# tuanggolt/hyperdrive

Measured on AMD Instinct MI355X. Metric: verified consensus msgs/sec (secp256k1) at 1/2/4/8 MI355X; % INT32 VALU peak, higher is better.
Workload: dtype u32 (256-bit modular integer arithmetic)

## Files before the change

### hyperdrive_amd/_lib.py

```python
from __future__ import annotations

import atexit
import ctypes
import os
import weakref

HERE = os.path.dirname(os.path.abspath(__file__))
LIB_PATH = os.environ.get("HD_LIB", os.path.join(HERE, "_lib", "libhdverify.so"))

HD_OK = 0
HD_EINVAL = -1
HD_ENOMEM = -2
HD_EDEVICE = -3
HD_ECAP = -4
HD_EAGAIN = -5

c_u8p = ctypes.POINTER(ctypes.c_uint8)
c_i8p = ctypes.POINTER(ctypes.c_int8)
c_i64p = ctypes.POINTER(ctypes.c_int64)
c_u32p = ctypes.POINTER(ctypes.c_uint32)
c_i32p = ctypes.POINTER(ctypes.c_int32)


class HdBatch(ctypes.Structure):
# ... 144 lines not shown
class HdMqTaken(ctypes.Structure):
    _fields_ = [("n", ctypes.c_uint32), ("removed", ctypes.c_uint32), ("batch", HdBatch),
                ("d_sender", ctypes.c_void_p), ("d_valid_bitmap", ctypes.c_void_p), ("d_value_ok", ctypes.c_void_p),
                ("n_proposes", ctypes.c_uint32), ("proposes", ctypes.c_void_p)]


class HdTallyTicket(ctypes.Structure):
    _fields_ = [("stage", ctypes.c_void_p), ("stage_cap", ctypes.c_size_t), ("dup", ctypes.c_int),
                ("n", ctypes.c_uint32), ("H", ctypes.c_uint32), ("Cg", ctypes.c_uint32), ("need", ctypes.c_size_t),
                ("done", ctypes.c_void_p)]


SIGNATURES = {
    "hd_ctx_create": (ctypes.c_int, [ctypes.c_int, ctypes.POINTER(ctypes.c_void_p)]),
    "hd_ctx_destroy": (ctypes.c_int, [ctypes.c_void_p]),
    "hd_ctx_set_pubkey_format": (ctypes.c_int, [ctypes.c_void_p, ctypes.c_int]),
    "hd_set_signatories": (ctypes.c_int, [ctypes.c_void_p, ctypes.c_void_p, ctypes.c_uint32]),
    "hd_import_keys": (ctypes.c_int, [ctypes.c_void_p, ctypes.c_void_p, ctypes.c_uint32, ctypes.c_void_p,
                                      ctypes.c_void_p]),
    "hd_export_keys": (ctypes.c_int, [ctypes.c_void_p, ctypes.c_void_p, ctypes.c_void_p, ctypes.c_uint32,
                                      ctypes.POINTER(ctypes.c_uint32)]),
    "hd_ctx_set_change_info": (ctypes.c_int, [ctypes.c_void_p, ctypes.POINTER(HdSetChangeInfo)]),
    "hd_ctx_set_fastpath": (ctypes.c_int, [ctypes.c_void_p, ctypes.c_int]),
    "hd_ctx_fastpath_stats": (ctypes.c_int, [ctypes.c_void_p, ctypes.POINTER(ctypes.c_uint32),
                                             ctypes.POINTER(ctypes.c_uint32)]),
    "hd_ctx_foreign_stats": (ctypes.c_int, [ctypes.c_void_p, ctypes.POINTER(ctypes.c_uint32),
                                            ctypes.POINTER(ctypes.c_uint32), ctypes.POINTER(ctypes.c_uint32)]),
    "hd_ctx_dedup_stats": (ctypes.c_int, [ctypes.c_void_p, ctypes.POINTER(ctypes.c_uint64),
                                          ctypes.POINTER(ctypes.c_uint64)]),
    "hd_ctx_preimage_stats": (ctypes.c_int, [ctypes.c_void_p, ctypes.POINTER(ctypes.c_uint64),
                                             ctypes.POINTER(ctypes.c_uint64)]),
    "hd_ctx_overlap_stats": (ctypes.c_int, [ctypes.c_void_p, ctypes.POINTER(ctypes.c_uint32),
                                            ctypes.POINTER(ctypes.c_uint32), ctypes.POINTER(ctypes.c_uint32)]),
    "hd_ctx_fastpath_geometry": (ctypes.c_int, [ctypes.c_void_p, ctypes.POINTER(ctypes.c_int),
                                                ctypes.POINTER(ctypes.c_int), ctypes.POINTER(ctypes.c_int)]),
    "hd_ctx_profile": (ctypes.c_int, [ctypes.c_void_p, ctypes.c_int]),
    "hd_ctx_set_variant": (ctypes.c_int, [ctypes.c_void_p, ctypes.c_int, ctypes.c_int]),
    "hd_ctx_get_variant": (ctypes.c_int, [ctypes.c_void_p, ctypes.c_int, ctypes.POINTER(ctypes.c_int)]),
    "hd_ctx_profile_read": (ctypes.c_int, [ctypes.c_void_p, ctypes.POINTER(ctypes.c_uint32),
                                           ctypes.POINTER(ctypes.c_double), ctypes.POINTER(ctypes.c_uint32),
                                           ctypes.POINTER(ctypes.c_double)]),
    "hd_verify_batch": (ctypes.c_int, [ctypes.c_void_p, ctypes.POINTER(HdBatch), ctypes.c_void_p,
                                       ctypes.c_void_p, ctypes.c_void_p]),
    "hd_verify_batch_device": (ctypes.c_int, [ctypes.c_void_p, ctypes.POINTER(HdBatch), ctypes.c_void_p,
                                              ctypes.c_void_p, ctypes.c_void_p, ctypes.c_void_p, ctypes.c_void_p]),
    "hd_authenticate_batch_device": (ctypes.c_int, [ctypes.c_void_p, ctypes.POINTER(HdBatch), ctypes.c_void_p,
                                                    ctypes.c_void_p]),
    "hd_verify_submit": (ctypes.c_int, [ctypes.c_void_p, ctypes.POINTER(HdBatch), ctypes.c_void_p, ctypes.c_void_p,
                                        ctypes.c_void_p, ctypes.POINTER(ctypes.c_uint64)]),
    "hd_verify_submit_compact": (ctypes.c_int, [ctypes.c_void_p, ctypes.POINTER(HdBatchCompact), ctypes.c_void_p,
                                                ctypes.c_void_p, ctypes.c_void_p, ctypes.POINTER(ctypes.c_uint64)]),
    "hd_verify_wait": (ctypes.c_int, [ctypes.c_void_p, ctypes.c_uint64]),
    "hd_host_alloc": (ctypes.c_int, [ctypes.c_size_t, ctypes.POINTER(ctypes.c_void_p)]),
    "hd_host_free": (ctypes.c_int, [ctypes.c_void_p]),
    "hd_stream_create_dedicated": (ctypes.c_int, [ctypes.c_void_p, ctypes.POINTER(ctypes.c_void_p)]),
    "hd_stream_destroy": (ctypes.c_int, [ctypes.c_void_p, ctypes.c_void_p]),
    "hd_tally": (ctypes.c_int, [ctypes.c_void_p, ctypes.POINTER(HdBatch), ctypes.c_void_p,
                                ctypes.POINTER(HdTallyOut)]),
    "hd_tally_device": (ctypes.c_int, [ctypes.c_void_p, ctypes.POINTER(HdBatch), ctypes.c_void_p,
                                       ctypes.POINTER(HdTallyOut), ctypes.c_void_p]),
    "hd_tally_device_bitmap_part": (ctypes.c_int, [ctypes.c_void_p, ctypes.POINTER(HdBatch), ctypes.c_void_p,
                                                   ctypes.c_uint32, ctypes.c_uint32, ctypes.POINTER(HdTallyOut),
                                                   ctypes.c_void_p]),
    "hd_tally_partition_of": (ctypes.c_uint32, [ctypes.c_int64, ctypes.c_int64, ctypes.c_uint32]),
    "hd_tally_device_bitmap": (ctypes.c_int, [ctypes.c_void_p, ctypes.POINTER(HdBatch), ctypes.c_void_p,
                                              ctypes.POINTER(HdTallyOut), ctypes.c_void_p]),
# ... 209 lines not shown
```

### hyperdrive_amd/csrc/hd_fastverify.hip

```cpp
#include <hip/hip_runtime.h>

#include <algorithm>
#include <cstdio>
#include <cstdlib>
#include <cstring>
#include <string>
#include <map>
#include <mutex>
#include <unordered_map>
#include <vector>

#include "../../include/hd_verify.h"
#include "../../include/hd_mathcheck.h"
#include "hd_fixedbase.h"
#include "hd_dedup.h"
#include "hd_scmont.h"
#include "hd_internal.h"
#include "hd_keycarry.h"
#include "hd_verify_msg.h"

using namespace hd;

struct FbWork {
    const gp* gtab = nullptr;
    uint32_t nslots = 0;
    uint32_t max_slots = 0;
    gp** tabs = nullptr;
    std::vector<gp*> chunks;
    ge* base = nullptr;
    ge* pub = nullptr;
    uint32_t* state = nullptr;
    int32_t* adm_slot = nullptr;
    bool map_ok = true;
    size_t cap_adm_slot = 0;
    uint32_t* list = nullptr;
    uint32_t* counts = nullptr;
    uint32_t* zr = nullptr;
    struct Scratch {
        uint32_t* rows = nullptr;
        size_t cap_rows = 0;
        uint32_t* dtab = nullptr;
        size_t cap_dtab = 0;
        uint8_t* pre = nullptr;
        size_t cap_pre = 0;
        uint32_t* slow = nullptr;
        size_t cap_slow = 0;
        uint32_t* count = nullptr;
        uint32_t* slow2 = nullptr;
        size_t cap_slow2 = 0;
        hipEvent_t done = nullptr;
        hipStream_t stream = nullptr;
        bool used = false;
    };
    static constexpr int NSCRATCH = 3;
    Scratch sc[NSCRATCH];
    int next = 0;
    int last_set = -1;
    uint32_t* nr_host = nullptr;
    uint32_t* nr_dev = nullptr;
    uint32_t* est_host = nullptr;
    uint32_t* est_dev = nullptr;
    unsigned long long* dstats = nullptr;
    unsigned long long* pstats = nullptr;
    hipEvent_t done = nullptr;
    hipStream_t last = nullptr;
    bool any = false;
    bool steady = false;
    struct SumsChain {
        hipEvent_t done = nullptr;
        hipStream_t last = nullptr;
        bool prev = false, now = false;
        void begin_call() { prev = now; now = false; }
        bool wait(hipStream_t s) {
            if (!done && hipEventCreateWithFlags(&done, hipEventDisableTiming) != hipSuccess) done = nullptr;
            return done && prev && last != s && hipStreamWaitEvent(s, done, 0) == hipSuccess;
        }
        void record(hipStream_t s) {
            now = done && hipEventRecord(done, s) == hipSuccess;
            if (now) last = s;
        }
    } sums;
    uint32_t n_capped = 0, n_lean = 0, n_chained = 0;
    bool prof = false;
    std::vector<hipEvent_t> ev_call, ev_sums;
    size_t n_call = 0, n_sums = 0;
    std::unordered_map<std::string, uint32_t> slot_of;
    std::vector<uint32_t> free_slots;
    hd_set_change_info change{0, 0, 0, 0, 0};
    uint32_t used = 1;
    int wp = HD_FB_W;
    int last_k = 8;
    double budget = 0;
    size_t bytes = 0;
    uint32_t* fdict = nullptr;
    uint32_t* fnext = nullptr;
    uint32_t fbase = 0, fcap = 0, fres = 0;
    uint32_t* fpend_host = nullptr;
    uint32_t* fpend_dev = nullptr;
    uint32_t fseen = 0;
    uint32_t* fhit = nullptr;
    ge* fkey = nullptr;
    uint32_t fwait = 1, fcalls = 0;
    bool fforce = false;
    uint32_t evictions = 0;
    uint32_t evict_checks = 0;
    uint32_t evict_aborts = 0;
};

namespace {

#define FBCHK(expr, what)                                \
    do {                                                 \
        hipError_t e_ = (expr);                          \
        if (e_ != hipSuccess) return hd_ctx_fail(ctx, e_, what); \
    } while (0)

struct FastSrc {
    const DevBatch& b;
    uint32_t i;
    const uint8_t* dg;
    __device__ __forceinline__ uint32_t type() const { return b.type[i]; }
    __device__ __forceinline__ uint32_t value(int w) const { return load_be32(b.value32 + 32 * (size_t)i + 4 * w); }
    __device__ __forceinline__ uint32_t from(int w) const { return load_be32(b.from32 + 32 * (size_t)i + 4 * w); }
    __device__ __forceinline__ uint32_t sig_r(int w) const { return load_be32(b.sig65 + 65 * (size_t)i + 4 * w); }
    __device__ __forceinline__ uint32_t sig_s(int w) const { return load_be32(b.sig65 + 65 * (size_t)i + 32 + 4 * w); }
    __device__ __forceinline__ uint32_t sig_v() const { return b.sig65[65 * (size_t)i + 64]; }
    __device__ __forceinline__ void sig(uint32_t r_be[8], uint32_t s_be[8], uint32_t& v) const {
        load_sig65(r_be, s_be, v, b.sig65, i, b.n);
    }
    __device__ __forceinline__ void from_words(uint32_t w[8]) const { load_row32_be(w, b.from32, i); }
    __device__ __forceinline__ void value_words(uint32_t w[8]) const { load_row32_be(w, b.value32, i); }
};

#define HD_FAST_LIVE 0xFDu

template <int NW>
HD void soa_load(uint32_t (&w)[NW], const uint32_t* __restrict__ p, uint32_t n, uint32_t i) {
    HD_UNROLL for (int k = 0; k < NW; k++) w[k] = p[(size_t)k * n + i];
}
template <int NW>
HD void soa_store(uint32_t* __restrict__ p, uint32_t n, uint32_t i, const uint32_t (&w)[NW]) {
    HD_UNROLL for (int k = 0; k < NW; k++) p[(size_t)k * n + i] = w[k];
}

struct SplitRows {
    uint32_t* aux;
    int32_t* idx;
    uint32_t* ref;
    uint32_t* u1;
    uint32_t* u2;
    uint32_t* s;
    uint32_t* pre;
    uint32_t* xyz;
    uint32_t* cnt;
    int prio;
};

HD uint32_t dd_resolve(const SplitRows& rows, uint32_t i, uint32_t& c, bool& has_slot) {
    uint32_t rf = rows.ref[i];
    has_slot = (rf >> 30) != 3u;
    c = 0;
    if (!has_slot) return rf & 0xFFu;
    if (rf & HD_DD_REPEAT) rf = rows.ref[rf & HD_DD_INDEX];
    c = rf;
    return rows.aux[c] & 0xFFu;
}

HD void wave_prio(int p) {
    if (p == 1) __builtin_amdgcn_s_setprio(1);
    else if (p == 2) __builtin_amdgcn_s_setprio(2);
    else if (p >= 3) __builtin_amdgcn_s_setprio(3);
}

#define HD_REF_NEG 0x80000000u
#define HD_REF_ZERO 0x40000000u
#define HD_REF_IDX 0x3FFFFFFFu
// ... 198 lines not shown
            }
        }
    }
    const bool live = code == HD_FAST_LIVE;
    const bool distinct = live && rep == HD_DD_EMPTY;
    __shared__ uint32_t s_cnt[4], s_base;
    const uint32_t lane = threadIdx.x & 63u, wv = threadIdx.x >> 6;
    const unsigned long long bd = __ballot(distinct), br = __ballot(live && !distinct);
    if (lane == 0) s_cnt[wv] = (uint32_t)__popcll(bd) | (uint32_t)__popcll(br) << 16;
    __syncthreads();
    if (threadIdx.x == 0) {
        const uint32_t t = s_cnt[0] + s_cnt[1] + s_cnt[2] + s_cnt[3];
        s_base = 0;
        if (t)
            s_base = (uint32_t)atomicAdd((unsigned long long*)(rows.cnt + 2),
                                         (unsigned long long)(t & 0xFFFFu) | (unsigned long long)(t >> 16) << 32);
    }
    __syncthreads();
    if (!present) return;
    if (distinct) {
        uint32_t c = s_base + (uint32_t)__popcll(bd & ((1ull << lane) - 1ull));
        for (uint32_t w = 0; w < wv; w++) c += s_cnt[w] & 0xFFFFu;
        rows.aux[c] = slot << 8 | HD_FAST_LIVE;
        soa_store(rows.u1, n, c, m.v);
        soa_store(rows.u2, n, c, r.v);
        soa_store(rows.s, n, c, s.v);
        rows.ref[i] = c;
    } else {
        rows.ref[i] = live ? (HD_DD_REPEAT | rep) : (HD_DD_FINAL | code);
    }
    rows.idx[i] = idx;
}

template <int K>
HD uint32_t split_lanes(uint32_t nc) {
    return ((nc + (uint32_t)K - 1) / (uint32_t)K + 63u) & ~63u;
}

template <int K>
__global__ __launch_bounds__(256) void k_fast_sinv(uint32_t n, SplitRows rows, uint32_t* __restrict__ est,
                                                   unsigned long long* __restrict__ stats) {
    wave_prio(rows.prio);
    const uint32_t t = blockIdx.x * blockDim.x + threadIdx.x;
    const uint32_t nc = rows.cnt[2], T = split_lanes<K>(nc);
    if (t == 0) {
        const uint32_t reps = rows.cnt[3];
        if (est) {
            est[1] = n;
            est[0] = nc;
        }
        if (nc + reps) atomicAdd(&stats[0], (unsigned long long)nc + reps);
        if (reps) atomicAdd(&stats[1], (unsigned long long)reps);
    }
    if (t >= T) return;
    sc sv[K];
    uint32_t live = 0;
    static_for<K>([&](auto jc) {
        constexpr int j = decltype(jc)::value;
        const uint32_t i = (uint32_t)j * T + t;
        const uint32_t ic = i < nc ? i : nc - 1;
        const uint32_t a = rows.aux[ic];
        soa_load(sv[j].v, rows.s, n, ic);
        live |= (i < nc && (a & 0xFFu) == HD_FAST_LIVE) ? 1u << j : 0u;
    });
    if (!live) return;
    sm pre[K], acc;
    HD_UNROLL for (int k = 0; k < 9; k++) acc.n[k] = 0;
    static_for<K>([&](auto jc) {
        constexpr int j = decltype(jc)::value;
        if ((live >> j) & 1u) {
// ... 260 lines not shown
    const uint32_t* zrow = rows.xyz + 18 * (size_t)n;
    uint32_t live = 0;
    fe acc;
    HD_UNROLL for (int k = 0; k < 9; k++) acc.n[k] = 0;
    HD_NOUNROLL for (int j = 0; j < K; j++) {
        const uint32_t i = (uint32_t)j * T + t;
        if (!lean_live(rows, nc, i)) continue;
        fe z;
        soa_load(z.n, zrow, n, i);
        if (live) fe_mul(acc, acc, z);
        else acc = z;
        live |= 1u << j;
        soa_store(rows.pre, n, i, acc.n);
    }
    if (!live) return;
    fe inv;
    fe_inv_divsteps(inv, acc);
    HD_NOUNROLL for (int j = K - 1; j >= 0; j--) {
        if (!((live >> j) & 1u)) continue;
        const uint32_t i = (uint32_t)j * T + t;
        const uint32_t below = live & ((1u << j) - 1u);
        if (below) {
            const uint32_t ip = (uint32_t)(31 - __clz((int)below)) * T + t;
            fe pp, zi, z;
            soa_load(pp.n, rows.pre, n, ip);
            soa_load(z.n, zrow, n, i);
            fe_mul(zi, inv, pp);
            fe_mul(inv, inv, z);
            soa_store(rows.pre, n, i, zi.n);
        } else {
            soa_store(rows.pre, n, i, inv.n);
        }
    }
}

HD void fast_rx(fe& x, const sc& r, uint32_t v) {
    uint32_t xw[8];
    HD_UNROLL for (int k = 0; k < 8; k++) xw[k] = r.v[k];
    if (v & 2) {
        const uint32_t N[8] = {HD_N0, HD_N1, HD_N2, HD_N3, HD_N4, 0xFFFFFFFFu, 0xFFFFFFFFu, 0xFFFFFFFFu};
        uint64_t c = 0;
        HD_UNROLL for (int k = 0; k < 8; k++) { c += (uint64_t)xw[k] + N[k]; xw[k] = (uint32_t)c; c >>= 32; }
    }
    fe_from_le(x, xw);
}

__device__ __forceinline__ void cmp_one(const DevBatch& b, const SplitRows& rows, const int32_t* __restrict__ adm_perm,
                       uint8_t* __restrict__ verdict, uint8_t* __restrict__ rec32, int32_t* __restrict__ signer,
                       uint32_t* __restrict__ slow, uint32_t* __restrict__ n_slow, uint32_t* __restrict__ bitmap,
                       bool auth, uint32_t i, bool present, const fe* zi) {
    const uint32_t n = b.n;
    uint8_t v = HD_NEEDS_SLOW;
    if (present) {
        uint32_t c;
        bool has_slot;
        v = (uint8_t)dd_resolve(rows, i, c, has_slot);
        if (v == HD_FAST_LIVE) {
            fe xn, yn, w, x;
            soa_load(xn.n, rows.xyz, n, c);
            soa_load(yn.n, rows.xyz + 9 * (size_t)n, n, c);
            if (zi) w = *zi;
            else soa_load(w.n, rows.pre, n, c);
            sc r;
            soa_load(r.v, rows.u2, n, c);
            const uint32_t sv = b.sig65[65 * (size_t)i + 64];
            fast_rx(x, r, sv);
// ... 483 lines not shown
    gp** tp = nullptr;
    ge *base = nullptr, *pub = nullptr;
    uint32_t* cl = nullptr;
    FBCHK(hipMalloc(&tab, sizeof(gp) * (size_t)FbL<HD_FB_WG>::TAB), "G table");
    FBCHK(hipMalloc(&tp, sizeof(gp*)), "G table pointer");
    FBCHK(hipMalloc(&base, sizeof(ge) * FbL<HD_FB_WG>::NWIN), "G bases");
    FBCHK(hipMalloc(&pub, sizeof(ge)), "G point");
    FBCHK(hipMalloc(&cl, 8), "G list");
    const uint32_t hl[2] = {0u, 1u};
    hipStream_t s = ctx->stream;
    FBCHK(hipMemcpyAsync(pub, &g, sizeof(ge), hipMemcpyHostToDevice, s), "G point");
    FBCHK(hipMemcpyAsync(cl, hl, 8, hipMemcpyHostToDevice, s), "G list");
    FBCHK(hipMemcpyAsync(tp, &tab, sizeof(gp*), hipMemcpyHostToDevice, s), "G table pointer");
    k_fb_bases<HD_FB_WG><<<1, 64, 0, s>>>(cl, cl + 1, pub, base);
    k_fb_runs<HD_FB_WG><<<fb_run_blocks(ctx), 256, 0, s>>>(cl, cl + 1, base, tp, ctx->fb->zr);
    FBCHK(hipGetLastError(), "G table kernels");
    FBCHK(hipStreamSynchronize(s), "G table build");
    (void)hipFree(base);
    (void)hipFree(pub);
    (void)hipFree(cl);
    (void)hipFree(tp);
    g_fb_g_tables[ctx->device] = tab;
    *out = tab;
    return HD_OK;
}

int hd_fb_init(hd_ctx* ctx) {
    if (ctx->fb) return HD_OK;
    ctx->fb = new (std::nothrow) FbWork();
    if (!ctx->fb) return HD_ENOMEM;
    FbWork* f = ctx->fb;
    f->budget = 64.0 * (1ull << 30);
    if (const char* m = getenv("HD_FB_MAX_BYTES")) f->budget = atof(m);
    f->max_slots = (uint32_t)std::max(1.0, std::min(1e6, f->budget / fb_slot_bytes(f->wp)));
    FBCHK(hipMalloc(&f->counts, 8), "fb counts");
    FBCHK(hipMalloc(&f->zr, fb_run_scratch_bytes(ctx)), "fb builder scratch");
    FBCHK(hipHostMalloc((void**)&f->nr_host, 4, hipHostMallocMapped | hipHostMallocCoherent), "fb ready count");
    *f->nr_host = 0xFFFFFFFFu;
    FBCHK(hipHostGetDevicePointer((void**)&f->nr_dev, f->nr_host, 0), "fb ready count map");
    FBCHK(hipHostMalloc((void**)&f->est_host, 16, hipHostMallocMapped | hipHostMallocCoherent), "fb list estimate");
    f->est_host[0] = f->est_host[1] = f->est_host[2] = f->est_host[3] = 0xFFFFFFFFu;
    FBCHK(hipHostGetDevicePointer((void**)&f->est_dev, f->est_host, 0), "fb list estimate map");
    FBCHK(hipHostMalloc((void**)&f->fpend_host, 8, hipHostMallocMapped | hipHostMallocCoherent), "fb foreign claims");
    f->fpend_host[0] = f->fpend_host[1] = 0;
    FBCHK(hipHostGetDevicePointer((void**)&f->fpend_dev, f->fpend_host, 0), "fb foreign claims map");
    FBCHK(hipMalloc(&f->dstats, 16), "fb repeat counters");
    FBCHK(hipMemset(f->dstats, 0, 16), "fb repeat counters clear");
    FBCHK(hipMalloc(&f->pstats, 16), "fb preimage counters");
    FBCHK(hipMemset(f->pstats, 0, 16), "fb preimage counters clear");
    int rc = fb_alloc_slots(ctx);
    if (rc) return rc;
    return fb_g_table(ctx, &f->gtab);
}

const gp* hd_fb_gtab(const hd_ctx* ctx) { return ctx && ctx->fb ? ctx->fb->gtab : nullptr; }

void hd_fb_release(hd_ctx* ctx) {
    if (!ctx || !ctx->fb) return;
    FbWork* f = ctx->fb;
    fb_free_tables(ctx);
    if (f->done) (void)hipEventDestroy(f->done);
    if (f->sums.done) (void)hipEventDestroy(f->sums.done);
    for (hipEvent_t e : f->ev_call) (void)hipEventDestroy(e);
    for (hipEvent_t e : f->ev_sums) (void)hipEventDestroy(e);
    for (auto& sc : f->sc) {
        if (sc.done) (void)hipEventDestroy(sc.done);
        void* sp[] = {sc.rows, sc.slow, sc.count, sc.slow2, sc.dtab, sc.pre};
        for (void* p : sp)
            if (p) (void)hipFree(p);
    }
    void* ptrs[] = {f->counts, f->adm_slot, f->zr, f->fdict, f->fnext, f->fhit, f->fkey, f->dstats, f->pstats};
    for (void* p : ptrs)
        if (p) (void)hipFree(p);
    if (f->nr_host) (void)hipHostFree(f->nr_host);
    if (f->est_host) (void)hipHostFree(f->est_host);
    if (f->fpend_host) (void)hipHostFree(f->fpend_host);
    delete f;
    ctx->fb = nullptr;
}

static double fb_free_cap(hd_ctx* ctx) {
    size_t fr = 0, tot = 0;
    (void)hipSetDevice(ctx->device);
    if (hipMemGetInfo(&fr, &tot) != hipSuccess) return 1e300;
    return 0.9 * (double)fr + (double)ctx->fb->bytes;
}

static int fb_pick_width(hd_ctx* ctx, uint32_t m, int cap) {
    if (ctx->var[HD_VAR_KEY_WIDTH]) return ctx->var[HD_VAR_KEY_WIDTH];
    FbWork* f = ctx->fb;
    const double others = (double)(fb_device_bytes(ctx->device) - std::min(fb_device_bytes(ctx->device), f->bytes));
    const double free_cap = fb_free_cap(ctx);
    const double shared = std::min(f->budget - others, free_cap);
    const double slots = (double)m + 1 + (ctx->var[HD_VAR_FOREIGN_KEYS] > 0 ? ctx->var[HD_VAR_FOREIGN_KEYS] : 0);
    const auto allowed = [cap](int w) { return cap == 0 || w <= cap; };
    if (allowed(HD_FB_WX) && fb_slot_bytes(HD_FB_WX) * slots <= shared) return HD_FB_WX;
    if (allowed(HD_FB_WW) && fb_slot_bytes(HD_FB_WW) * ((double)m + 1) <= shared) return HD_FB_WW;
    if (allowed(HD_FB_W) && fb_slot_bytes(HD_FB_W) * slots <= std::min(f->budget, free_cap)) return HD_FB_W;
    return HD_FB_WN;
}
// ... 261 lines not shown
static void launch_sums(const FbCallPlan& p, uint32_t blocks, hipStream_t s, uint32_t n, const gp* gtab,
                        const gp* const* tab, const SplitRows& rows) {
    const size_t cap = p.capped ? sums_cap_lds<WP>() : 0;
    if (p.sums_pf == 2) {
        if (p.sums_waves == 2) k_fast_sums<2, WP, 2><<<blocks, 256, 0, s>>>(n, gtab, tab, rows);
        else k_fast_sums<3, WP, 2><<<blocks, 256, cap, s>>>(n, gtab, tab, rows);
    } else {
        if (p.sums_waves == 2) k_fast_sums<2, WP, 1><<<blocks, 256, 0, s>>>(n, gtab, tab, rows);
        else if (p.sums_waves == 4) k_fast_sums<4, WP, 0><<<blocks, 256, 0, s>>>(n, gtab, tab, rows);
        else k_fast_sums<3, WP, 1><<<blocks, 256, cap, s>>>(n, gtab, tab, rows);
    }
}

template <int K, int WP>
static void launch_split(hd_ctx* ctx, const DevBatch& b, const uint8_t* d_digest, uint8_t* d_verdict,
                         uint8_t* d_rec32, int32_t* d_signer, uint32_t* d_bitmap, const SplitRows& rows,
                         const FbWork::Scratch& sc, hipStream_t s, bool auth, const FbCallPlan& p) {
    FbWork* f = ctx->fb;
    const uint32_t n = b.n;
    const uint32_t tb = (split_lanes<K>(n) + 255) / 256, nb = (n + 255) / 256;
    const uint32_t tw = dd_table_words(n);
    uint32_t* dtab = p.dedup ? sc.dtab : nullptr;
    const uint32_t* fdict = f->fcap ? f->fdict : nullptr;
    if (p.share) {
        const PreRows pre{sc.pre, (uint32_t*)(sc.pre + 32 * (size_t)n), (uint32_t*)(sc.pre + 36 * (size_t)n), sc.count};
        k_pre_claim<<<(n + HD_PRE_BLOCK - 1) / HD_PRE_BLOCK, HD_PRE_BLOCK, 0, s>>>(b, pre, sc.dtab + tw, tw - 1u, rows.prio);
        k_pre_hash<<<nb, 256, 0, s>>>(b, pre, f->pstats, rows.prio);
        k_fast_prep<true><<<nb, 256, 0, s>>>(b, nullptr, f->state, f->adm_slot, hd_adm_index(ctx), ctx->n_adm, rows,
                                             fdict, f->fhit, f->fbase, dtab, tw - 1u, pre);
    } else {
        k_fast_prep<false><<<nb, 256, 0, s>>>(b, d_digest, f->state, f->adm_slot, hd_adm_index(ctx), ctx->n_adm, rows,
                                              fdict, f->fhit, f->fbase, dtab, tw - 1u, PreRows{});
    }
    if (p.lean) k_fast_sinv_lean<K><<<tb, 256, 0, s>>>(n, rows, f->est_dev + 2, f->dstats);
    else k_fast_sinv<K><<<tb, 256, 0, s>>>(n, rows, f->est_dev + 2, f->dstats);
    if (p.chain && f->sums.wait(s)) f->n_chained++;
    hipEvent_t* pe = fb_prof_pair(f->ev_sums, f->n_sums, f->prof);
    if (pe) (void)hipEventRecord(pe[0], s);
    launch_sums<WP>(p, nb, s, n, f->gtab, f->tabs, rows);
    if (pe) (void)hipEventRecord(pe[1], s);
    if (p.chain) f->sums.record(s);
    if (p.lean) k_fast_zinv_lean<K><<<tb, 256, 0, s>>>(n, rows);
    else k_fast_zinv<K><<<tb, 256, 0, s>>>(n, rows);
    k_fast_cmp<<<nb, 256, 0, s>>>(b, rows, ctx->d_adm_perm, d_verdict, d_rec32, d_signer, sc.slow, sc.count,
                                  d_bitmap, auth);
}

static int fb_verify_impl(hd_ctx* ctx, const DevBatch& b, const uint8_t* d_digest, uint8_t* d_verdict,
                          uint8_t* d_rec32, int32_t* d_signer, uint32_t* d_bitmap, FbWork::Scratch& sc,
                          hipStream_t s, bool auth);

int hd_fb_verify(hd_ctx* ctx, const DevBatch& b, const uint8_t* d_digest, uint8_t* d_verdict, uint8_t* d_rec32,
                 int32_t* d_signer, uint32_t* d_bitmap, hipStream_t s, bool auth) {
    FbWork* f = ctx->fb;
    f->sums.begin_call();
    if (!f->done) FBCHK(hipEventCreateWithFlags(&f->done, hipEventDisableTiming), "fb event");
    const int j = f->next;
    f->next = (j + 1) % FbWork::NSCRATCH;
    FbWork::Scratch& sc = f->sc[j];
    if (!sc.done) FBCHK(hipEventCreateWithFlags(&sc.done, hipEventDisableTiming), "fb scratch event");
    if (!sc.count) FBCHK(hipMalloc(&sc.count, 32), "fb scratch count");
    bool evicted = false;
    int re = fb_evict(ctx, &evicted);
    if (re) return re;
    const bool steady = !evicted && f->nr_host && *(volatile uint32_t*)f->nr_host == 0 && !fb_foreign_pending(f);
    if (sc.used && sc.stream != s) FBCHK(hipStreamWaitEvent(s, sc.done, 0), "fb scratch order");
    if (f->any && f->last != s && !(steady && f->steady)) FBCHK(hipStreamWaitEvent(s, f->done, 0), "fb stream order");
    hipEvent_t* pe = fb_prof_pair(f->ev_call, f->n_call, f->prof);
    if (pe) (void)hipEventRecord(pe[0], s);
    const int rc = fb_verify_impl(ctx, b, d_digest, d_verdict, d_rec32, d_signer, d_bitmap, sc, s, auth);
    if (pe) (void)hipEventRecord(pe[1], s);
    FBCHK(hipEventRecord(sc.done, s), "fb scratch record");
    FBCHK(hipEventRecord(f->done, s), "fb event record");
    sc.used = true;
    sc.stream = s;
    f->last_set = j;
// ... 15 lines not shown
static int fb_verify_impl(hd_ctx* ctx, const DevBatch& b, const uint8_t* d_digest, uint8_t* d_verdict,
                          uint8_t* d_rec32, int32_t* d_signer, uint32_t* d_bitmap, FbWork::Scratch& sc,
                          hipStream_t s, bool auth) {
    FbWork* f = ctx->fb;
    int rc = hd_dev_grow(ctx, (void**)&sc.slow, &sc.cap_slow, 4 * (size_t)b.n);
    if (rc) return rc;
    const uint32_t blocks = (b.n + 255) / 256;
    rc = hd_dev_grow(ctx, (void**)&sc.slow2, &sc.cap_slow2, 4 * (size_t)b.n);
    if (rc) return rc;
    FBCHK(hipMemsetAsync(sc.count, 0, 32, s), "fb count reset");
    if (ctx->n_adm > 0 && f->adm_slot && f->map_ok) {
        if (b.n > HD_DD_MAX_N) {
            ctx->last_error = "known-key check: more than 2^30 messages in one call";
            return HD_EINVAL;
        }
        const size_t row_words = 63;
        rc = hd_dev_grow(ctx, (void**)&sc.rows, &sc.cap_rows, 4 * row_words * (size_t)b.n);
        if (rc) return rc;
        const uint32_t n = b.n;
        const volatile uint32_t* est = f->est_host;
        const FbCallPlan p = fb_plan_call(FbPlanIn{ctx->var, ctx->n_cu, n, auth, d_digest != nullptr,
                                                   {est[0], est[1], est[2], est[3]}});
        if (p.dedup || p.share) {
            const size_t tab_bytes = 4 * (size_t)dd_table_words(n);
            rc = hd_dev_grow(ctx, (void**)&sc.dtab, &sc.cap_dtab, 2 * tab_bytes);
            if (rc) return rc;
            const size_t first = p.dedup ? 0 : tab_bytes, last = p.share ? 2 * tab_bytes : tab_bytes;
            FBCHK(hipMemsetAsync((uint8_t*)sc.dtab + first, 0xFF, last - first, s), "fb table clear");
        }
        if (p.share) {
            rc = hd_dev_grow(ctx, (void**)&sc.pre, &sc.cap_pre, 40 * (size_t)n);
            if (rc) return rc;
        }
        SplitRows rows;
        rows.aux = sc.rows;
        rows.idx = (int32_t*)(sc.rows + (size_t)n);
        rows.u1 = sc.rows + 2 * (size_t)n;
        rows.u2 = sc.rows + 10 * (size_t)n;
        rows.s = sc.rows + 18 * (size_t)n;
        rows.pre = sc.rows + 26 * (size_t)n;
        rows.xyz = sc.rows + 35 * (size_t)n;
        rows.ref = sc.rows + 62 * (size_t)n;
        rows.cnt = sc.count;
        rows.prio = ctx->var[HD_VAR_WAVE_PRIO];
        with_width(f->wp, [&](auto wp) {
            with_k(p.k, [&](auto k) {
                launch_split<decltype(k)::value, decltype(wp)::value>(ctx, b, d_digest, d_verdict, d_rec32, d_signer,
                                                                      d_bitmap, rows, sc, s, auth, p);
            });
        });
        f->last_k = p.k;
        f->n_capped += p.capped;
        f->n_lean += p.lean;
        FBCHK(hipGetLastError(), "split check launch");
        if (p.lift) {
            k_slow_lift<<<p.lift_blocks, 256, 0, s>>>(b, sc.slow, sc.count, d_verdict, d_rec32, d_signer, sc.slow2,
                                                      sc.count + 1, rows.prio, f->est_dev, rows, f->gtab);
            FBCHK(hipGetLastError(), "k_slow_lift");
        }
        const SlowCtl ctl{p.lift ? sc.slow2 : sc.slow, p.lift ? sc.count + 1 : sc.count, f->adm_slot, f->state, f->pub,
                          d_bitmap, p.lift ? f->est_dev + 1 : f->est_dev, rows.prio,
                          f->fcap ? f->fdict : nullptr, f->fnext, f->fbase, f->fcap, f->fpend_dev,
                          f->fcap ? f->fhit + 64 : nullptr, f->fkey, f->fpend_dev + 1};
        rc = hd_launch_slow(ctx, b, d_digest, d_verdict, d_rec32, d_signer, nullptr, ctl, p.slow_blocks, s);
        if (rc) return rc;
        return fb_learn(ctx, s);
// ... 112 lines not shown
int hd_ctx_set_change_info(hd_ctx* ctx, hd_set_change_info* out) {
    if (!ctx || !out) return HD_EINVAL;
    *out = ctx->fb && ctx->fastpath ? ctx->fb->change : hd_set_change_info{0, 0, 0, 0, 0};
    return HD_OK;
}

int hd_ctx_dedup_stats(hd_ctx* ctx, uint64_t* checked, uint64_t* repeats) {
    if (!ctx) return HD_EINVAL;
    if (checked) *checked = 0;
    if (repeats) *repeats = 0;
    if (!ctx->fb || !ctx->fb->dstats) return HD_OK;
    (void)hipSetDevice(ctx->device);
    int rq = hd_ctx_quiesce(ctx);
    if (rq) return rq;
    unsigned long long st[2] = {0, 0};
    FBCHK(hipMemcpy(st, ctx->fb->dstats, 16, hipMemcpyDeviceToHost), "repeat counters read");
    if (checked) *checked = st[0];
    if (repeats) *repeats = st[1];
    return HD_OK;
}

int hd_ctx_preimage_stats(hd_ctx* ctx, uint64_t* typed, uint64_t* distinct) {
    if (!ctx) return HD_EINVAL;
    if (typed) *typed = 0;
    if (distinct) *distinct = 0;
    if (!ctx->fb || !ctx->fb->pstats) return HD_OK;
    (void)hipSetDevice(ctx->device);
    int rq = hd_ctx_quiesce(ctx);
    if (rq) return rq;
    unsigned long long st[2] = {0, 0};
    FBCHK(hipMemcpy(st, ctx->fb->pstats, 16, hipMemcpyDeviceToHost), "preimage counters read");
    if (typed) *typed = st[0];
    if (distinct) *distinct = st[1];
    return HD_OK;
}

int hd_ctx_overlap_stats(hd_ctx* ctx, uint32_t* capped, uint32_t* lean, uint32_t* chained) {
    if (!ctx) return HD_EINVAL;
    const FbWork* f = ctx->fb;
    if (capped) *capped = f ? f->n_capped : 0;
    if (lean) *lean = f ? f->n_lean : 0;
    if (chained) *chained = f ? f->n_chained : 0;
    return HD_OK;
}

int hd_fb_table_read(hd_ctx* ctx, int32_t which, uint64_t first, uint32_t count, uint8_t* out64, int* width,
                     uint32_t* state, uint8_t* key64) {
    if (!ctx || !ctx->fb || which < -1 || (count && !out64)) return HD_EINVAL;
    (void)hipSetDevice(ctx->device);
    FbWork* f = ctx->fb;
    int rq = hd_fb_quiesce(ctx);
    if (rq) return rq;
    FBCHK(hipStreamSynchronize(ctx->stream), "table read sync");
    const gp* tab = nullptr;
    uint64_t entries = 0;
    uint32_t st = HD_FB_READY;
    int w = HD_FB_WG;
    gp key;
    if (which < 0) {
        ge g;
        const uint32_t GX[8] = {0x79BE667Eu, 0xF9DCBBACu, 0x55A06295u, 0xCE870B07u,
                                0x029BFCDBu, 0x2DCE28D9u, 0x59F2815Bu, 0x16F81798u};
        const uint32_t GY[8] = {0x483ADA77u, 0x26A3C465u, 0x5DA4FBFCu, 0x0E1108A8u,
                                0xFD17B448u, 0xA6855419u, 0x9C47D08Fu, 0xFB10D4B8u};
        fe_from_be(g.x, GX);
        fe_from_be(g.y, GY);
// ... 37 lines not shown
```

### hyperdrive_amd/verify.py

```python
from __future__ import annotations

import ctypes
from dataclasses import dataclass
from typing import Dict, List, Optional, Sequence, Tuple

import numpy as np

from . import _lib
from ._lib import HDError, HdBatch, HdTallyOut

VALID = 0
BAD_RECID = 1
BAD_RS = 2
NO_POINT = 3
INFINITY = 4
SIGNATORY_MISMATCH = 5
NOT_ADMITTED = 6
BAD_TYPE = 7
NOT_AUTHENTIC = 8
VERDICT_NAMES = ["VALID", "BAD_RECID", "BAD_RS", "NO_POINT", "INFINITY", "SIGNATORY_MISMATCH",
                 "NOT_ADMITTED", "BAD_TYPE", "NOT_AUTHENTIC"]

PROPOSE, PREVOTE, PRECOMMIT = 1, 2, 3

# ... 726 lines not shown
        self._check(self._lib.hd_ctx_profile_read(self._ctx, ctypes.byref(c), ctypes.byref(vm), ctypes.byref(s),
                                                  ctypes.byref(sm)), "hd_ctx_profile_read")
        return c.value, vm.value, s.value, sm.value

    def fastpath_stats(self) -> Tuple[int, int]:
        k, f = ctypes.c_uint32(), ctypes.c_uint32()
        self._check(self._lib.hd_ctx_fastpath_stats(self._ctx, ctypes.byref(k), ctypes.byref(f)),
                    "hd_ctx_fastpath_stats")
        return int(k.value), int(f.value)

    def foreign_stats(self, checks: bool = False):
        r, e, c = ctypes.c_uint32(), ctypes.c_uint32(), ctypes.c_uint32()
        self._check(self._lib.hd_ctx_foreign_stats(self._ctx, ctypes.byref(r), ctypes.byref(e), ctypes.byref(c)),
                    "hd_ctx_foreign_stats")
        return (int(r.value), int(e.value), int(c.value)) if checks else (int(r.value), int(e.value))

    def dedup_stats(self) -> Tuple[int, int]:
        c, r = ctypes.c_uint64(), ctypes.c_uint64()
        self._check(self._lib.hd_ctx_dedup_stats(self._ctx, ctypes.byref(c), ctypes.byref(r)), "hd_ctx_dedup_stats")
        return int(c.value), int(r.value)

    def preimage_stats(self) -> Tuple[int, int]:
        t, d = ctypes.c_uint64(), ctypes.c_uint64()
        self._check(self._lib.hd_ctx_preimage_stats(self._ctx, ctypes.byref(t), ctypes.byref(d)),
                    "hd_ctx_preimage_stats")
        return int(t.value), int(d.value)

    def overlap_stats(self) -> Tuple[int, int, int]:
        c, l, w = ctypes.c_uint32(), ctypes.c_uint32(), ctypes.c_uint32()
        self._check(self._lib.hd_ctx_overlap_stats(self._ctx, ctypes.byref(c), ctypes.byref(l), ctypes.byref(w)),
                    "hd_ctx_overlap_stats")
        return int(c.value), int(l.value), int(w.value)

    def fastpath_geometry(self) -> Tuple[int, int, int]:
        g, k, m = ctypes.c_int(), ctypes.c_int(), ctypes.c_int()
        self._check(self._lib.hd_ctx_fastpath_geometry(self._ctx, ctypes.byref(g), ctypes.byref(k), ctypes.byref(m)),
                    "hd_ctx_fastpath_geometry")
        return int(g.value), int(k.value), int(m.value)

    def known_keys(self) -> int:
        return self.fastpath_stats()[0]

    def verify_batch(self, batch: Batch, recovered: bool = True) -> VerifyResult:
        n = len(batch)
        verdict = np.zeros(n, np.uint8)
        rec = np.zeros((n, 32), np.uint8)
        bitmap = np.zeros((n + 31) // 32, np.uint32)
        cb = batch.c_struct()
        self._check(self._lib.hd_verify_batch(self._ctx, ctypes.byref(cb), _ptr(verdict),
                                              _ptr(rec) if recovered else None, _ptr(bitmap)), "hd_verify_batch")
        return VerifyResult(verdict, rec, bitmap)

    def submit(self, batch: Batch, verdict: np.ndarray, recovered: Optional[np.ndarray] = None,
               bitmap: Optional[np.ndarray] = None) -> int:
        cb = batch.c_struct()
        t = ctypes.c_uint64()
        self._check(self._lib.hd_verify_submit(self._ctx, ctypes.byref(cb), _ptr(verdict), _ptr(recovered),
                                               _ptr(bitmap), ctypes.byref(t)), "hd_verify_submit")
        return t.value

    def submit_compact(self, batch: CompactBatch, verdict: np.ndarray, recovered: Optional[np.ndarray] = None,
                       bitmap: Optional[np.ndarray] = None) -> int:
        cb = batch.c_struct()
        t = ctypes.c_uint64()
        self._check(self._lib.hd_verify_submit_compact(self._ctx, ctypes.byref(cb), _ptr(verdict), _ptr(recovered),
                                                       _ptr(bitmap), ctypes.byref(t)), "hd_verify_submit_compact")
# ... 297 lines not shown
```

### include/hd_verify.h

```cpp
#ifndef HD_VERIFY_H
#define HD_VERIFY_H

#include <stddef.h>
#include <stdint.h>

#ifdef __cplusplus
extern "C" {
#endif

#define HD_OK 0
#define HD_EINVAL (-1)
#define HD_ENOMEM (-2)
#define HD_EDEVICE (-3)
#define HD_ECAP (-4)
#define HD_EAGAIN (-5)

#define HD_TYPE_PROPOSE 1
#define HD_TYPE_PREVOTE 2
#define HD_TYPE_PRECOMMIT 3

#define HD_VERDICT_VALID 0
#define HD_VERDICT_BAD_RECID 1
#define HD_VERDICT_BAD_RS 2
#define HD_VERDICT_NO_POINT 3
// ... 14 lines not shown
    const uint8_t* value32;
    const uint8_t* from32;
    const uint8_t* sig65;
} hd_batch;

int hd_ctx_create(int device, hd_ctx** out);
int hd_ctx_destroy(hd_ctx* ctx);
#define HD_PUBKEY_UNCOMPRESSED 0
#define HD_PUBKEY_COMPRESSED 1
#define HD_PUBKEY_RAW64 2
#define HD_PUBKEY_XY_STRIPPED 3
int hd_ctx_set_pubkey_format(hd_ctx* ctx, int format);
int hd_set_signatories(hd_ctx* ctx, const uint8_t* sigs32, uint32_t n);
typedef struct {
    int width_before, width_after;
    uint32_t kept;
    uint32_t carried;
    uint32_t dropped;
} hd_set_change_info;
int hd_ctx_set_change_info(hd_ctx* ctx, hd_set_change_info* out);
#define HD_KEY_IMPORTED     0
#define HD_KEY_KNOWN        1
#define HD_KEY_NOT_ADMITTED 2
#define HD_KEY_NO_SLOT      3
#define HD_KEY_BAD_POINT    4
int hd_import_keys(hd_ctx* ctx, const uint8_t* keys64, uint32_t n, uint8_t* status, int32_t* signer);
int hd_export_keys(hd_ctx* ctx, uint8_t* keys64, uint8_t* known, uint32_t cap, uint32_t* n_out);
int hd_ctx_set_fastpath(hd_ctx* ctx, int enable);
int hd_ctx_fastpath_stats(hd_ctx* ctx, uint32_t* known_keys, uint32_t* last_fallback);
int hd_ctx_foreign_stats(hd_ctx* ctx, uint32_t* ready_slots, uint32_t* evictions, uint32_t* checks);
int hd_ctx_dedup_stats(hd_ctx* ctx, uint64_t* checked, uint64_t* repeats);
int hd_ctx_preimage_stats(hd_ctx* ctx, uint64_t* typed, uint64_t* distinct);
int hd_ctx_overlap_stats(hd_ctx* ctx, uint32_t* capped, uint32_t* lean, uint32_t* chained);
int hd_ctx_fastpath_geometry(hd_ctx* ctx, int* g_windows, int* key_windows, int* msgs_per_inversion);
int hd_ctx_profile(hd_ctx* ctx, int enable);
#define HD_VAR_VERIFY_WAVES 0
#define HD_VAR_SUM_WAVES 1
#define HD_VAR_SUM_PREFETCH 2
#define HD_VAR_SPLIT_K 4
#define HD_VAR_RECOVER_G 5
#define HD_VAR_KEY_WIDTH 7
#define HD_VAR_WAVE_PRIO 8
#define HD_VAR_FOREIGN_KEYS 10
#define HD_VAR_SLOW_LIFT 11
#define HD_VAR_DEDUP 12
#define HD_VAR_PRE_SHARE 15
#define HD_VAR_SUM_CAP 9
#define HD_VAR_LEAN_INV 13
#define HD_VAR_SUM_CHAIN 14
#define HD_VAR__COUNT 16
int hd_ctx_set_variant(hd_ctx* ctx, int which, int value);
int hd_ctx_get_variant(hd_ctx* ctx, int which, int* value);
int hd_ctx_profile_read(hd_ctx* ctx, uint32_t* calls, double* verify_ms, uint32_t* sums_launches, double* sums_ms);

int hd_verify_batch(hd_ctx* ctx, const hd_batch* batch, uint8_t* verdict, uint8_t* recovered32,
                    uint32_t* valid_bitmap);

int hd_verify_batch_device(hd_ctx* ctx, const hd_batch* dbatch, uint8_t* d_verdict, uint8_t* d_recovered32,
                           int32_t* d_signer, uint32_t* d_valid_bitmap, void* stream);

int hd_authenticate_batch_device(hd_ctx* ctx, const hd_batch* dbatch, uint8_t* d_verdict, void* stream);

#define HD_HOST_SLOTS 3
int hd_verify_submit(hd_ctx* ctx, const hd_batch* batch, uint8_t* verdict, uint8_t* recovered32,
                     uint32_t* valid_bitmap, uint64_t* ticket);
int hd_verify_wait(hd_ctx* ctx, uint64_t ticket);
// ... 180 lines not shown
```

Baseline: 1.061 billion.

## Add two-level batched modular inversion with separate up/mid/down kernels

Replaces the single-level Montgomery batch inversion for scalar (s) and Z coordinate inverses with a two-level tree. An up kernel builds per-lane prefix products and writes lane roots, a mid kernel batches K2 roots per thread and does one modular inversion per group, and a down kernel propagates inverses back. The goal is to cut the number of expensive divstep inversions by a further factor of K2. The cost is extra kernel launches, root buffers and memory traffic. It is enabled by default on the lean path, with env and API switches to fall back.

```diff
diff --git a/hyperdrive_amd/_lib.py b/hyperdrive_amd/_lib.py
--- a/hyperdrive_amd/_lib.py
+++ b/hyperdrive_amd/_lib.py
@@ -200,6 +200,8 @@
                                              ctypes.POINTER(ctypes.c_uint64)]),
     "hd_ctx_overlap_stats": (ctypes.c_int, [ctypes.c_void_p, ctypes.POINTER(ctypes.c_uint32),
                                             ctypes.POINTER(ctypes.c_uint32), ctypes.POINTER(ctypes.c_uint32)]),
+    "hd_ctx_inv_levels": (ctypes.c_int, [ctypes.c_void_p, ctypes.c_int]),
+    "hd_ctx_inv_stats": (ctypes.c_int, [ctypes.c_void_p, ctypes.POINTER(ctypes.c_uint64)]),
     "hd_ctx_fastpath_geometry": (ctypes.c_int, [ctypes.c_void_p, ctypes.POINTER(ctypes.c_int),
                                                 ctypes.POINTER(ctypes.c_int), ctypes.POINTER(ctypes.c_int)]),
     "hd_ctx_profile": (ctypes.c_int, [ctypes.c_void_p, ctypes.c_int]),
diff --git a/hyperdrive_amd/csrc/hd_fastverify.hip b/hyperdrive_amd/csrc/hd_fastverify.hip
--- a/hyperdrive_amd/csrc/hd_fastverify.hip
+++ b/hyperdrive_amd/csrc/hd_fastverify.hip
@@ -15,6 +15,7 @@
 #include "hd_fixedbase.h"
 #include "hd_dedup.h"
 #include "hd_scmont.h"
+#include "hd_inv2.h"
 #include "hd_internal.h"
 #include "hd_keycarry.h"
 #include "hd_verify_msg.h"
@@ -39,6 +40,8 @@
     struct Scratch {
         uint32_t* rows = nullptr;
         size_t cap_rows = 0;
+        uint32_t* roots = nullptr;
+        size_t cap_roots = 0;
         uint32_t* dtab = nullptr;
         size_t cap_dtab = 0;
         uint8_t* pre = nullptr;
@@ -81,6 +84,8 @@
         }
     } sums;
     uint32_t n_capped = 0, n_lean = 0, n_chained = 0;
+    int inv_levels = 2, inv_k2 = 16;
+    uint64_t n_inv[2] = {0, 0};
     bool prof = false;
     std::vector<hipEvent_t> ev_call, ev_sums;
     size_t n_call = 0, n_sums = 0;
@@ -132,16 +137,6 @@
     __device__ __forceinline__ void value_words(uint32_t w[8]) const { load_row32_be(w, b.value32, i); }
 };
 
-#define HD_FAST_LIVE 0xFDu
-
-template <int NW>
-HD void soa_load(uint32_t (&w)[NW], const uint32_t* __restrict__ p, uint32_t n, uint32_t i) {
-    HD_UNROLL for (int k = 0; k < NW; k++) w[k] = p[(size_t)k * n + i];
-}
-template <int NW>
-HD void soa_store(uint32_t* __restrict__ p, uint32_t n, uint32_t i, const uint32_t (&w)[NW]) {
-    HD_UNROLL for (int k = 0; k < NW; k++) p[(size_t)k * n + i] = w[k];
-}
 
 struct SplitRows {
     uint32_t* aux;
@@ -406,10 +401,6 @@
     rows.idx[i] = idx;
 }
 
-template <int K>
-HD uint32_t split_lanes(uint32_t nc) {
-    return ((nc + (uint32_t)K - 1) / (uint32_t)K + 63u) & ~63u;
-}
 
 template <int K>
 __global__ __launch_bounds__(256) void k_fast_sinv(uint32_t n, SplitRows rows, uint32_t* __restrict__ est,
@@ -736,6 +727,76 @@
             soa_store(rows.pre, n, i, inv.n);
         }
     }
+}
+
+struct RootRows {
+    uint32_t* roots;
+    uint32_t* rpre;
+};
+
+template <int K>
+__global__ __launch_bounds__(256, 3) void k_fast_sinv_up(uint32_t n, SplitRows rows, RootRows rr,
+                                                         uint32_t* __restrict__ est,
+                                                         unsigned long long* __restrict__ stats) {
+    wave_prio(rows.prio);
+    const uint32_t t = blockIdx.x * blockDim.x + threadIdx.x;
+    const uint32_t nc = rows.cnt[2], T = split_lanes<K>(nc);
+    if (t == 0) {
+        const uint32_t reps = rows.cnt[3];
+        if (est) {
+            est[1] = n;
+            est[0] = nc;
+        }
+        if (nc + reps) atomicAdd(&stats[0], (unsigned long long)nc + reps);
+        if (reps) atomicAdd(&stats[1], (unsigned long long)reps);
+    }
+    if (t >= T) return;
+    inv2_up<sm, K>(t, T, nc, n, rows.aux, rows.s, rows.pre, rr.roots);
+}
+
+template <int K2, int K>
+__global__ __launch_bounds__(256, 3) void k_fast_sinv_mid(SplitRows rows, RootRows rr) {
+    wave_prio(rows.prio);
+    const uint32_t u = blockIdx.x * blockDim.x + threadIdx.x;
+    const uint32_t T = split_lanes<K>(rows.cnt[2]), T2 = split_lanes<K2>(T);
+    if (u >= T2) return;
+    inv2_mid<sm, K2>(u, T2, T, rr.roots, rr.rpre);
+}
+
+template <int K>
+__global__ __launch_bounds__(256, 3) void k_fast_sinv_down(uint32_t n, SplitRows rows, RootRows rr) {
+    wave_prio(rows.prio);
+    const uint32_t t = blockIdx.x * blockDim.x + threadIdx.x;
+    const uint32_t nc = rows.cnt[2], T = split_lanes<K>(nc);
+    if (t >= T) return;
+    inv2_down<sm, K>(t, T, nc, n, rows.aux, rows.s, rows.pre, rr.roots);
+}
+
+template <int K>
+__global__ __launch_bounds__(256, 3) void k_fast_zinv_up(uint32_t n, SplitRows rows, RootRows rr) {
+    wave_prio(rows.prio);
+    const uint32_t t = blockIdx.x * blockDim.x + threadIdx.x;
+    const uint32_t nc = rows.cnt[2], T = split_lanes<K>(nc);
+    if (t >= T) return;
+    inv2_up<fe, K>(t, T, nc, n, rows.aux, rows.xyz + 18 * (size_t)n, rows.pre, rr.roots);
+}
+
+template <int K2, int K>
+__global__ __launch_bounds__(256, 3) void k_fast_zinv_mid(SplitRows rows, RootRows rr) {
+    wave_prio(rows.prio);
+    const uint32_t u = blockIdx.x * blockDim.x + threadIdx.x;
+    const uint32_t T = split_lanes<K>(rows.cnt[2]), T2 = split_lanes<K2>(T);
+    if (u >= T2) return;
+    inv2_mid<fe, K2>(u, T2, T, rr.roots, rr.rpre);
+}
+
+template <int K>
+__global__ __launch_bounds__(256, 3) void k_fast_zinv_down(uint32_t n, SplitRows rows, RootRows rr) {
+    wave_prio(rows.prio);
+    const uint32_t t = blockIdx.x * blockDim.x + threadIdx.x;
+    const uint32_t nc = rows.cnt[2], T = split_lanes<K>(nc);
+    if (t >= T) return;
+    inv2_down<fe, K>(t, T, nc, n, rows.aux, rows.xyz + 18 * (size_t)n, rows.pre, rr.roots);
 }
 
 HD void fast_rx(fe& x, const sc& r, uint32_t v) {
@@ -1285,6 +1346,8 @@
     FbWork* f = ctx->fb;
     f->budget = 64.0 * (1ull << 30);
     if (const char* m = getenv("HD_FB_MAX_BYTES")) f->budget = atof(m);
+    if (const char* l = getenv("HD_INV_LEVELS")) f->inv_levels = atoi(l) == 1 ? 1 : 2;
+    if (const char* k2 = getenv("HD_INV_K2")) f->inv_k2 = atoi(k2) == 8 ? 8 : 16;
     f->max_slots = (uint32_t)std::max(1.0, std::min(1e6, f->budget / fb_slot_bytes(f->wp)));
     FBCHK(hipMalloc(&f->counts, 8), "fb counts");
     FBCHK(hipMalloc(&f->zr, fb_run_scratch_bytes(ctx)), "fb builder scratch");
@@ -1318,7 +1381,7 @@
     for (hipEvent_t e : f->ev_sums) (void)hipEventDestroy(e);
     for (auto& sc : f->sc) {
         if (sc.done) (void)hipEventDestroy(sc.done);
-        void* sp[] = {sc.rows, sc.slow, sc.count, sc.slow2, sc.dtab, sc.pre};
+        void* sp[] = {sc.rows, sc.slow, sc.count, sc.slow2, sc.dtab, sc.pre, sc.roots};
         for (void* p : sp)
             if (p) (void)hipFree(p);
     }
@@ -1646,7 +1709,17 @@
         k_fast_prep<false><<<nb, 256, 0, s>>>(b, d_digest, f->state, f->adm_slot, hd_adm_index(ctx), ctx->n_adm, rows,
                                               fdict, f->fhit, f->fbase, dtab, tw - 1u, PreRows{});
     }
-    if (p.lean) k_fast_sinv_lean<K><<<tb, 256, 0, s>>>(n, rows, f->est_dev + 2, f->dstats);
+    const bool two = p.lean && f->inv_levels == 2;
+    const uint32_t rt = split_lanes<8>(n);
+    const RootRows rr{sc.roots, two ? sc.roots + 9 * (size_t)rt : nullptr};
+    const bool k2w = f->inv_k2 == 8;
+    const uint32_t mb = ((k2w ? split_lanes<8>(split_lanes<K>(n)) : split_lanes<16>(split_lanes<K>(n))) + 255) / 256;
+    if (two) {
+        k_fast_sinv_up<K><<<tb, 256, 0, s>>>(n, rows, rr, f->est_dev + 2, f->dstats);
+        if (k2w) k_fast_sinv_mid<8, K><<<mb, 256, 0, s>>>(rows, rr);
+        else k_fast_sinv_mid<16, K><<<mb, 256, 0, s>>>(rows, rr);
+        k_fast_sinv_down<K><<<tb, 256, 0, s>>>(n, rows, rr);
+    } else if (p.lean) k_fast_sinv_lean<K><<<tb, 256, 0, s>>>(n, rows, f->est_dev + 2, f->dstats);
     else k_fast_sinv<K><<<tb, 256, 0, s>>>(n, rows, f->est_dev + 2, f->dstats);
     if (p.chain && f->sums.wait(s)) f->n_chained++;
     hipEvent_t* pe = fb_prof_pair(f->ev_sums, f->n_sums, f->prof);
@@ -1654,8 +1727,14 @@
     launch_sums<WP>(p, nb, s, n, f->gtab, f->tabs, rows);
     if (pe) (void)hipEventRecord(pe[1], s);
     if (p.chain) f->sums.record(s);
-    if (p.lean) k_fast_zinv_lean<K><<<tb, 256, 0, s>>>(n, rows);
+    if (two) {
+        k_fast_zinv_up<K><<<tb, 256, 0, s>>>(n, rows, rr);
+        if (k2w) k_fast_zinv_mid<8, K><<<mb, 256, 0, s>>>(rows, rr);
+        else k_fast_zinv_mid<16, K><<<mb, 256, 0, s>>>(rows, rr);
+        k_fast_zinv_down<K><<<tb, 256, 0, s>>>(n, rows, rr);
+    } else if (p.lean) k_fast_zinv_lean<K><<<tb, 256, 0, s>>>(n, rows);
     else k_fast_zinv<K><<<tb, 256, 0, s>>>(n, rows);
+    if (p.lean) f->n_inv[two ? 0 : 1]++;
     k_fast_cmp<<<nb, 256, 0, s>>>(b, rows, ctx->d_adm_perm, d_verdict, d_rec32, d_signer, sc.slow, sc.count,
                                   d_bitmap, auth);
 }
@@ -1737,6 +1816,10 @@
             rc = hd_dev_grow(ctx, (void**)&sc.pre, &sc.cap_pre, 40 * (size_t)n);
             if (rc) return rc;
         }
+        if (p.lean && f->inv_levels == 2) {
+            rc = hd_dev_grow(ctx, (void**)&sc.roots, &sc.cap_roots, 4 * 18 * (size_t)split_lanes<8>(n));
+            if (rc) return rc;
+        }
         SplitRows rows;
         rows.aux = sc.rows;
         rows.idx = (int32_t*)(sc.rows + (size_t)n);
@@ -1915,6 +1998,20 @@
     FBCHK(hipMemcpy(st, ctx->fb->pstats, 16, hipMemcpyDeviceToHost), "preimage counters read");
     if (typed) *typed = st[0];
     if (distinct) *distinct = st[1];
+    return HD_OK;
+}
+
+int hd_ctx_inv_levels(hd_ctx* ctx, int set) {
+    if (!ctx || !ctx->fb || (set != -1 && set != 1 && set != 2)) return HD_EINVAL;
+    if (set != -1) ctx->fb->inv_levels = set;
+    return ctx->fb->inv_levels;
+}
+
+int hd_ctx_inv_stats(hd_ctx* ctx, uint64_t out[2]) {
+    if (!ctx || !out) return HD_EINVAL;
+    const FbWork* f = ctx->fb;
+    out[0] = f ? f->n_inv[0] : 0;
+    out[1] = f ? f->n_inv[1] : 0;
     return HD_OK;
 }
 
diff --git a/hyperdrive_amd/csrc/hd_inv2.h b/hyperdrive_amd/csrc/hd_inv2.h
--- /dev/null
+++ b/hyperdrive_amd/csrc/hd_inv2.h
@@ -0,0 +1,135 @@
+#pragma once
+#include "hd_modinv.h"
+#include "hd_scmont.h"
+
+namespace hd {
+
+#define HD_FAST_LIVE 0xFDu
+
+template <int NW>
+HD void soa_load(uint32_t (&w)[NW], const uint32_t* __restrict__ p, uint32_t n, uint32_t i) {
+    HD_UNROLL for (int k = 0; k < NW; k++) w[k] = p[(size_t)k * n + i];
+}
+template <int NW>
+HD void soa_store(uint32_t* __restrict__ p, uint32_t n, uint32_t i, const uint32_t (&w)[NW]) {
+    HD_UNROLL for (int k = 0; k < NW; k++) p[(size_t)k * n + i] = w[k];
+}
+
+template <int K>
+HD uint32_t split_lanes(uint32_t nc) {
+    return ((nc + (uint32_t)K - 1) / (uint32_t)K + 63u) & ~63u;
+}
+
+HD void inv2_leaf(sm& x, const uint32_t* __restrict__ row, uint32_t n, uint32_t i) {
+    sc s;
+    soa_load(s.v, row, n, i);
+    sm_from_sc(x, s);
+}
+HD void inv2_mul(sm& r, const sm& a, const sm& b) { sm_mul(r, a, b); }
+HD void inv2_inv(sm& r, const sm& a) {
+    sc p, pinv;
+    sm_to_sc(p, a);
+    sc_inv_divsteps(pinv, p);
+    sm_from_sc(r, pinv);
+    sm r2;
+    sm_r2(r2);
+    sm_mul(r, r, r2);
+}
+HD void inv2_one(sm& r) {
+    sm u, r2;
+    HD_UNROLL for (int k = 0; k < 9; k++) u.n[k] = k == 0 ? 1u : 0u;
+    sm_r2(r2);
+    sm_mul(r, r2, u);
+}
+
+HD void inv2_leaf(fe& x, const uint32_t* __restrict__ row, uint32_t n, uint32_t i) { soa_load(x.n, row, n, i); }
+HD void inv2_mul(fe& r, const fe& a, const fe& b) { fe_mul(r, a, b); }
+HD void inv2_inv(fe& r, const fe& a) { fe_inv_divsteps(r, a); }
+HD void inv2_one(fe& r) {
+    HD_UNROLL for (int k = 0; k < 9; k++) r.n[k] = k == 0 ? 1u : 0u;
+}
+
+HD bool inv2_live(const uint32_t* __restrict__ aux, uint32_t nc, uint32_t i) {
+    return i < nc && (aux[i] & 0xFFu) == HD_FAST_LIVE;
+}
+
+template <class E, int K>
+HD void inv2_up(uint32_t t, uint32_t T, uint32_t nc, uint32_t n, const uint32_t* __restrict__ aux,
+                const uint32_t* __restrict__ in, uint32_t* __restrict__ pre, uint32_t* __restrict__ roots) {
+    uint32_t live = 0;
+    E acc;
+    HD_UNROLL for (int k = 0; k < 9; k++) acc.n[k] = 0;
+    HD_NOUNROLL for (int j = 0; j < K; j++) {
+        const uint32_t i = (uint32_t)j * T + t;
+        if (!inv2_live(aux, nc, i)) continue;
+        E x;
+        inv2_leaf(x, in, n, i);
+        if (live) inv2_mul(acc, acc, x);
+        else acc = x;
+        live |= 1u << j;
+        soa_store(pre, n, i, acc.n);
+    }
+    if (!live) inv2_one(acc);
+    soa_store(roots, T, t, acc.n);
+}
+
+template <class E, int K2>
+HD void inv2_mid(uint32_t u, uint32_t T2, uint32_t T, uint32_t* __restrict__ roots, uint32_t* __restrict__ rpre) {
+    int m = 0;
+    E acc;
+    HD_UNROLL for (int k = 0; k < 9; k++) acc.n[k] = 0;
+    HD_NOUNROLL for (int j = 0; j < K2; j++) {
+        const uint32_t r = (uint32_t)j * T2 + u;
+        if (r >= T) break;
+        E x;
+        soa_load(x.n, roots, T, r);
+        if (j) inv2_mul(acc, acc, x);
+        else acc = x;
+        m = j + 1;
+        soa_store(rpre, T, r, acc.n);
+    }
+    if (!m) return;
+    E inv;
+    inv2_inv(inv, acc);
+    HD_NOUNROLL for (int j = m - 1; j >= 0; j--) {
+        const uint32_t r = (uint32_t)j * T2 + u;
+        if (j) {
+            E pp, x, xi;
+            soa_load(pp.n, rpre, T, r - T2);
+            soa_load(x.n, roots, T, r);
+            inv2_mul(xi, inv, pp);
+            inv2_mul(inv, inv, x);
+            soa_store(roots, T, r, xi.n);
+        } else {
+            soa_store(roots, T, r, inv.n);
+        }
+    }
+}
+
+template <class E, int K>
+HD void inv2_down(uint32_t t, uint32_t T, uint32_t nc, uint32_t n, const uint32_t* __restrict__ aux,
+                  const uint32_t* __restrict__ in, uint32_t* __restrict__ pre, const uint32_t* __restrict__ roots) {
+    uint32_t live = 0;
+    HD_NOUNROLL for (int j = 0; j < K; j++) live |= inv2_live(aux, nc, (uint32_t)j * T + t) ? 1u << j : 0u;
+    if (!live) return;
+    E inv;
+    soa_load(inv.n, roots, T, t);
+    HD_NOUNROLL for (int j = K - 1; j >= 0; j--) {
+        if (!((live >> j) & 1u)) continue;
+        const uint32_t i = (uint32_t)j * T + t;
+        const uint32_t below = live & ((1u << j) - 1u);
+        if (below) {
+            const uint32_t ip = (uint32_t)(31 - __builtin_clz(below)) * T + t;
+            E pp, x, xi;
+            soa_load(pp.n, pre, n, ip);
+            inv2_leaf(x, in, n, i);
+            inv2_mul(xi, inv, pp);
+            inv2_mul(inv, inv, x);
+            soa_store(pre, n, i, xi.n);
+        } else {
+            soa_store(pre, n, i, inv.n);
+        }
+    }
+}
+
+}
diff --git a/hyperdrive_amd/verify.py b/hyperdrive_amd/verify.py
--- a/hyperdrive_amd/verify.py
+++ b/hyperdrive_amd/verify.py
@@ -782,6 +782,17 @@
                     "hd_ctx_overlap_stats")
         return int(c.value), int(l.value), int(w.value)
 
+    def inv_levels(self, set: int = -1) -> int:
+        got = self._lib.hd_ctx_inv_levels(self._ctx, set)
+        if got not in (1, 2):
+            self._check(got if got < 0 else -1, "hd_ctx_inv_levels")
+        return got
+
+    def inv_stats(self) -> Tuple[int, int]:
+        out = (ctypes.c_uint64 * 2)()
+        self._check(self._lib.hd_ctx_inv_stats(self._ctx, out), "hd_ctx_inv_stats")
+        return int(out[0]), int(out[1])
+
     def fastpath_geometry(self) -> Tuple[int, int, int]:
         g, k, m = ctypes.c_int(), ctypes.c_int(), ctypes.c_int()
         self._check(self._lib.hd_ctx_fastpath_geometry(self._ctx, ctypes.byref(g), ctypes.byref(k), ctypes.byref(m)),
diff --git a/include/hd_verify.h b/include/hd_verify.h
--- a/include/hd_verify.h
+++ b/include/hd_verify.h
@@ -70,6 +70,8 @@
 int hd_ctx_dedup_stats(hd_ctx* ctx, uint64_t* checked, uint64_t* repeats);
 int hd_ctx_preimage_stats(hd_ctx* ctx, uint64_t* typed, uint64_t* distinct);
 int hd_ctx_overlap_stats(hd_ctx* ctx, uint32_t* capped, uint32_t* lean, uint32_t* chained);
+int hd_ctx_inv_levels(hd_ctx* ctx, int set);
+int hd_ctx_inv_stats(hd_ctx* ctx, uint64_t out[2]);
 int hd_ctx_fastpath_geometry(hd_ctx* ctx, int* g_windows, int* key_windows, int* msgs_per_inversion);
 int hd_ctx_profile(hd_ctx* ctx, int enable);
 #define HD_VAR_VERIFY_WAVES 0
```

After: 1.091 billion, median of 6. +2.8%, better.
